# NVlabs/ODISE

Hardware: NVIDIA H100
Metric: images/sec @1024x1024 panoptic inference (ODISE hot path) (higher is better)
Workload: dtype f16q8

## Files before the change

include/odise_b200.h:

```cpp
#ifndef ODISE_B200_H_
#define ODISE_B200_H_

#include <stdint.h>

#ifdef __cplusplus
extern "C" {
#endif

#define ODISE_OK 0
#define ODISE_ERR_ARG 10001
#define ODISE_ERR_ALIGN 10002
#define ODISE_ERR_DRIVER 10003
#define ODISE_ERR_TENSORMAP 10004
#define ODISE_ERR_WORKSPACE 10005
#define ODISE_ERR_UNSUPPORTED 10006

#define ODISE_ACT_NONE 0
#define ODISE_ACT_RELU 1
#define ODISE_ACT_SILU 2
#define ODISE_ACT_GELU 3
#define ODISE_ACT_QUICKGELU 4

#define ODISE_PLANES_BF16 0
#define ODISE_PLANES_F16 1
// ... 77 lines not shown
  float alpha;
  const float* bias;
  const float* rowbias; int rows_per_group; long long rowbias_ld;
  int act;
  const float* residual; long long ld_residual; long long residual_batch_stride;
  float* out_f32; long long ld_out; long long out_batch_stride;
  void* out_hi; void* out_lo; long long ld_out_bf16; long long out_bf16_batch_stride;
  int split_k; void* workspace; long long workspace_bytes;
  int force_bn;
  const float* bias_m;
  int conv_mode;
  int geglu;
  float* gn_partial;
  long long gn_seg_stride; long long gn_plane_stride;
  int out_planes_fp16;
} odise_gemm_desc;
int odise_gemm_bf16(const odise_gemm_desc* desc, void* stream);
int odise_gemm_tile_policy(int M, int N, int K, int batch, int conv3x3, int nmma, int* bn, int* pair);
int odise_profile_begin(void);
int odise_profile_end(long long* launches, double* total_ms, double* total_flops);


int odise_split_f32(const float* x, long long ldx, void* hi, void* lo, long long ldo, long long rows, int cols,
                    void* stream);
int odise_split_f16_f32(const float* x, long long ldx, void* hi, void* lo, long long ldo, long long rows, int cols,
                        void* stream);
int odise_groupnorm_stats_f32(const float* x, long long ldx, float* mean, float* rstd, int B, int HW, int C, int G,
                              float eps, void* stream);
int odise_groupnorm_stats_bs_f32(const float* x, long long ldx, long long x_bs, float* mean, float* rstd, int B,
                                 int HW, int C, int G, float eps, void* stream);
long long odise_groupnorm_ws_floats(int B, int HW, int C, int G);
int odise_groupnorm_stats_ws_f32(const float* x, long long ldx, long long x_bs, float* ws, float* mean, float* rstd,
                                 int B, int HW, int C, int G, float eps, void* stream);
// ... 118 lines not shown
```

odise_b200/csrc/gemm_tc.cu:

```cuda
#include "ptx.cuh"
#include "wgmma.cuh"
#include "odise_b200.h"
#include "launch_count.h"
#include <cudaTypedefs.h>
#include <mutex>
#include <map>
#include <cstring>
#include <vector>
#include <cstdlib>
#include <cstdio>

namespace ob {

struct GemmParams {
  int M, N, K, batch;
  int a_batched, b_batched;
  int conv, C, H, W, bw, bh, bb;
  int nseg;
  int cstride, cpad;
  int tiles_m, tiles_n, splits, kblocks;
  float alpha;
  const float* bias;
  const float* bias_m;
  const float* rowbias;
// ... 162 lines not shown
template <int BN, int NMMA>
struct GemmCfg {
  static constexpr int BM = 128, BK = 64;
  static constexpr int A_BYTES = BM * BK * 2;
  static constexpr int B_BYTES = BN * BK * 2;
  static constexpr int PLANES = (NMMA == 1) ? 1 : 2;
  static constexpr int STAGE_BYTES = PLANES * (A_BYTES + B_BYTES);
  static constexpr int THREADS = 384;
  static constexpr int EPI_BYTES = 8 * 32 * 16 * 4;
  static constexpr int STAGES_RAW = (232448 - EPI_BYTES - 256 - 1024) / STAGE_BYTES;
  static constexpr int STAGES = STAGES_RAW > 8 ? 8 : STAGES_RAW;
  static constexpr int SMEM_BYTES = STAGES * STAGE_BYTES + EPI_BYTES + 256 + 1024;
  static_assert(STAGES >= 2, "GEMM tile does not fit shared memory");
};

template <int BN, int NMMA, int EPI>
__global__ void __launch_bounds__(GemmCfg<BN, NMMA>::THREADS, 1)
gemm_tc_kernel(const __grid_constant__ CUtensorMap tmAh, const __grid_constant__ CUtensorMap tmAl,
               const __grid_constant__ CUtensorMap tmBh, const __grid_constant__ CUtensorMap tmBl, const GemmParams p) {
  using Cfg = GemmCfg<BN, NMMA>;
  extern __shared__ uint8_t smem_raw[];
  uint8_t* smem = reinterpret_cast<uint8_t*>((reinterpret_cast<uintptr_t>(smem_raw) + 1023) & ~uintptr_t(1023));
  float* epi_smem = reinterpret_cast<float*>(smem + Cfg::STAGES * Cfg::STAGE_BYTES);
  uint64_t* bars = reinterpret_cast<uint64_t*>(smem + Cfg::STAGES * Cfg::STAGE_BYTES + Cfg::EPI_BYTES);
  uint64_t* full = bars;
  uint64_t* empty = bars + Cfg::STAGES;

  const int warp = threadIdx.x >> 5;
  const int lane = threadIdx.x & 31;

  if (warp == 8 && lane == 0) {
    tma_prefetch_desc(&tmAh);
    tma_prefetch_desc(&tmBh);
    if (NMMA != 1) {
      tma_prefetch_desc(&tmAl);
      tma_prefetch_desc(&tmBl);
    }
    for (int s = 0; s < Cfg::STAGES; ++s) {
      mbar_init(&full[s], 1);
      mbar_init(&empty[s], 8);
    }
    fence_barrier_init();
  }
  __syncthreads();

  const int tiles_per_z = p.tiles_m * p.tiles_n * p.splits;
  const int total_tiles = tiles_per_z * p.batch;
  const int kb_per_split = (p.kblocks + p.splits - 1) / p.splits;

  if (warp >= 8) {
    setmaxnreg_dec<40>();
    if (warp == 8 && lane == 0) {
      int stage = 0;
      uint32_t phase = 0;
      const int cpk = p.conv ? (p.C / 64) : 1;
      for (int tile = blockIdx.x; tile < total_tiles; tile += gridDim.x) {
        const int z = tile / tiles_per_z;
        int r = tile - z * tiles_per_z;
        const int sp = r / (p.tiles_m * p.tiles_n);
        r -= sp * (p.tiles_m * p.tiles_n);
        const int mt = r / p.tiles_n, nt = r % p.tiles_n;
        const int m0 = mt * 128, n0 = nt * BN;
        const int kb0 = sp * kb_per_split;
        const int kb1 = min(p.kblocks, kb0 + kb_per_split);
        int b0 = 0, h0 = 0, w0 = 0;
        if (p.conv) {
          const int hw = p.H * p.W;
          b0 = m0 / hw;
          const int rem = m0 - b0 * hw;
          h0 = rem / p.W;
          w0 = rem - h0 * p.W;
        }
        for (int kb = kb0; kb < kb1; ++kb) {
          mbar_wait(&empty[stage], phase ^ 1);
          uint8_t* st = smem + stage * Cfg::STAGE_BYTES;
          mbar_arrive_expect_tx(&full[stage], Cfg::STAGE_BYTES);
// ... 4 lines not shown
              const int cx = w0 * p.cstride + kw - p.cpad, cy = h0 * p.cstride + kh - p.cpad;
              tma_load_4d(st, &tmAh, &full[stage], cc * 64, cx, cy, b0);
              if (NMMA != 1) tma_load_4d(st + Cfg::A_BYTES, &tmAl, &full[stage], cc * 64, cx, cy, b0);
            } else {
              const int hw = p.H * p.W;
              for (int sg = 0; sg < p.nseg; ++sg) {
                const int m = m0 + sg * p.bw;
                const int bi = m / hw, rem = m - bi * hw;
                const int hi_ = rem / p.W, wi = rem - hi_ * p.W;
                const int cx = wi * p.cstride + kw - p.cpad, cy = hi_ * p.cstride + kh - p.cpad;
                uint8_t* sa = st + sg * p.bw * 128;
                tma_load_4d(sa, &tmAh, &full[stage], cc * 64, cx, cy, bi);
                if (NMMA != 1) tma_load_4d(sa + Cfg::A_BYTES, &tmAl, &full[stage], cc * 64, cx, cy, bi);
              }
            }
          } else {
            const int za = p.a_batched ? z : 0;
            tma_load_3d(st, &tmAh, &full[stage], kb * 64, m0, za);
            if (NMMA != 1) tma_load_3d(st + Cfg::A_BYTES, &tmAl, &full[stage], kb * 64, m0, za);
          }
          const int zb = p.b_batched ? z : 0;
          uint8_t* sb = st + Cfg::PLANES * Cfg::A_BYTES;
          tma_load_3d(sb, &tmBh, &full[stage], kb * 64, n0, zb);
          if (NMMA != 1) tma_load_3d(sb + Cfg::B_BYTES, &tmBl, &full[stage], kb * 64, n0, zb);
          if (++stage == Cfg::STAGES) { stage = 0; phase ^= 1; }
        }
      }
    }
    return;
  }

  setmaxnreg_inc<232>();
  const int wg = warp >> 2, wi = warp & 3;
  int stage = 0;
  uint32_t phase = 0;
  float acc[BN / 2];
  float acc2[BN / 2];
  float* stg_wg = epi_smem + wg * (4 * 512);
  float* stg = stg_wg + wi * 512;
  const int cq = lane & 3, rsub = lane >> 2;
  for (int tile = blockIdx.x; tile < total_tiles; tile += gridDim.x) {
    const int z = tile / tiles_per_z;
    int r = tile - z * tiles_per_z;
    const int sp = r / (p.tiles_m * p.tiles_n);
    r -= sp * (p.tiles_m * p.tiles_n);
    const int mt = r / p.tiles_n, nt = r % p.tiles_n;
    const int n0 = nt * BN;
    const int kb0 = sp * kb_per_split;
    const int kb1 = min(p.kblocks, kb0 + kb_per_split);

    if (kb0 >= kb1) {
#pragma unroll
      for (int i = 0; i < BN / 2; ++i) acc[i] = 0.f;
      if constexpr (NMMA == 2) {
#pragma unroll
        for (int i = 0; i < BN / 2; ++i) acc2[i] = 0.f;
      }
    }
    int prev = -1;
    for (int kb = kb0; kb < kb1; ++kb) {
      mbar_wait(&full[stage], phase);
// ... 12 lines not shown
        if constexpr (NMMA == 3) {
          wgmma_bf16(acc, a_hi, wgmma_desc_sw128(sb + Cfg::B_BYTES + k * 32), 1);
          wgmma_bf16(acc, wgmma_desc_sw128(sa + Cfg::A_BYTES + k * 32), b_hi, 1);
        }
      }
      if constexpr (NMMA == 2) {
        const uint32_t a2 = sa + Cfg::A_BYTES, b2 = sb + Cfg::B_BYTES;
#pragma unroll
        for (int k = 0; k < 2; ++k) {
          wgmma_e5m2(acc2, wgmma_desc_sw128(a2 + k * 32), wgmma_desc_sw128(b2 + 64 + k * 32), (kb > kb0 || k > 0) ? 1 : 0);
          wgmma_e5m2(acc2, wgmma_desc_sw128(a2 + 64 + k * 32), wgmma_desc_sw128(b2 + k * 32), 1);
        }
      }
      wgmma_commit();
      wgmma_wait<1>();
      if (prev >= 0 && lane == 0) mbar_arrive(&empty[prev]);
      prev = stage;
      if (++stage == Cfg::STAGES) { stage = 0; phase ^= 1; }
    }
    wgmma_wait<0>();
    reg_fence(acc);
    if (prev >= 0 && lane == 0) mbar_arrive(&empty[prev]);
    if constexpr (NMMA == 2) {
      reg_fence(acc2);
#pragma unroll
      for (int i = 0; i < BN / 2; ++i) acc[i] += acc2[i];
    }

    const int m_base = mt * 128 + wg * 64 + (wi & 1) * 32;
    const bool interior = p.vec_ok && p.splits == 1 && (mt * 128 + 128 <= p.M) && (n0 + BN <= p.N);
    constexpr bool EXTRA = EPI == 1, GEGLU = EPI == 2;
    const bool has_bias = p.bias != nullptr, has_res = EXTRA && p.res != nullptr;
    const bool to_f32 = p.D != nullptr, to_hi = p.Dh != nullptr, to_lo = p.Dl != nullptr;
    const int act = p.act;
    const float alpha = p.alpha;
    const bool has_gn = !GEGLU && p.gnp != nullptr;
    const long long gn_seg = ((long long)z * p.M + m_base) >> 5;
// ... 162 lines not shown
  });
  return fn;
}

static int encode_map(CUtensorMap* tm, const void* base, int rank, const cuuint64_t* dims,
                      const cuuint64_t* strides_bytes, const cuuint32_t* box, int spatial_stride = 1) {
  auto enc = get_encode();
  if (!enc) return ODISE_ERR_DRIVER;
  cuuint32_t estr[5] = {1, (cuuint32_t)spatial_stride, (cuuint32_t)spatial_stride, 1, 1};
  CUresult r = enc(tm, CU_TENSOR_MAP_DATA_TYPE_BFLOAT16, rank, const_cast<void*>(base), dims, strides_bytes, box,
                   estr, CU_TENSOR_MAP_INTERLEAVE_NONE, CU_TENSOR_MAP_SWIZZLE_128B,
                   CU_TENSOR_MAP_L2_PROMOTION_L2_256B, CU_TENSOR_MAP_FLOAT_OOB_FILL_NONE);
  return r == CUDA_SUCCESS ? ODISE_OK : ODISE_ERR_TENSORMAP;
}

struct ProfRec { cudaEvent_t a, b; double flops; int M, N, K, batch, conv, bn, nmma, splits; };
static std::vector<ProfRec> g_prof;
static bool g_prof_on = false;

int num_sms() {
  static int n = 0;
  if (!n) {
    int dev = 0;
    cudaGetDevice(&dev);
    cudaDeviceGetAttribute(&n, cudaDevAttrMultiProcessorCount, dev);
    if (n <= 0) n = 132;
  }
  return n;
}

template <int BN, int NMMA, int EPI>
static int launch_cfg(const CUtensorMap& ah, const CUtensorMap& al, const CUtensorMap& bh, const CUtensorMap& bl,
                      const GemmParams& p, cudaStream_t stream) {
  using Cfg = GemmCfg<BN, NMMA>;
  static bool attr_set = false;
  if (!attr_set) {
    cudaError_t e = cudaFuncSetAttribute(gemm_tc_kernel<BN, NMMA, EPI>, cudaFuncAttributeMaxDynamicSharedMemorySize,
                                         Cfg::SMEM_BYTES);
    if (e != cudaSuccess) return (int)e;
    attr_set = true;
  }
  const int total = p.tiles_m * p.tiles_n * p.splits * p.batch;
  const int grid = total < num_sms() ? total : num_sms();
  gemm_tc_kernel<BN, NMMA, EPI><<<grid, Cfg::THREADS, Cfg::SMEM_BYTES, stream>>>(ah, al, bh, bl, p);
  return (int)cudaGetLastError();
}

static int pick_tile(int M, int N, int K, int batch, int forced, bool conv, int nmma) {
  const int cands[4] = {256, 160, 128, 64};
  const double eff[4] = {0.833, 0.933, 1.0, 1.333};
  const double epi_k = 480.0;
  const long long tm = (M + 127) / 128;
  double best = 1e30;
  int c = 128;
  for (int i = 0; i < 4; ++i) {
    const int bn = cands[i];
    if (forced && bn != forced) continue;
    if (nmma == 2 && bn > 128) continue;
    const long long tn = (N + bn - 1) / bn;
    const long long units = tm * tn * batch;
    const long long waves = (units + num_sms() - 1) / num_sms();
    double cost;
    if (conv) {
      cost = (double)waves * bn * eff[i] + 0.02 * bn;
    } else {
      const double mma = (double)bn * K * eff[i], epi = (double)bn * epi_k;
      cost = (double)waves * ((mma > epi ? mma : epi) + 20000.0);
    }
    if (cost < best) { best = cost; c = bn; }
  }
  return c;
}

}

using namespace ob;

extern "C" int odise_gemm_bf16(const odise_gemm_desc* d, void* stream_v) {
  cudaStream_t stream = reinterpret_cast<cudaStream_t>(stream_v);
  if (!d || !d->a_hi || !d->b_hi) return ODISE_ERR_ARG;
  if (d->nmma != 1 && d->nmma != 2 && d->nmma != 3) return ODISE_ERR_ARG;
  if (d->nmma != 1 && (!d->a_lo || !d->b_lo)) return ODISE_ERR_ARG;
  if (d->M <= 0 || d->N <= 0 || d->K <= 0 || d->batch <= 0) return ODISE_ERR_ARG;
  if (!d->out_f32 && !d->out_hi) return ODISE_ERR_ARG;

  GemmParams p{};
  p.M = d->M; p.N = d->N; p.K = d->K; p.batch = d->batch;
  p.a_batched = d->a_batch_stride != 0; p.b_batched = d->b_batch_stride != 0;
  p.conv = d->conv3x3; p.C = d->conv_C; p.H = d->conv_H; p.W = d->conv_W;
  p.alpha = d->alpha;
  p.bias = d->bias; p.bias_m = d->bias_m; p.rowbias = d->rowbias; p.rows_per_group = d->rows_per_group > 0 ? d->rows_per_group : 1;
  p.rowbias_ld = d->rowbias_ld;
  p.res = d->residual; p.ldres = d->ld_residual; p.res_bs = d->residual_batch_stride;
  p.D = d->out_f32; p.ldd = d->ld_out; p.d_bs = d->out_batch_stride;
  p.Dh = reinterpret_cast<__nv_bfloat16*>(d->out_hi); p.Dl = reinterpret_cast<__nv_bfloat16*>(d->out_lo);
  p.ldh = d->ld_out_bf16; p.h_bs = d->out_bf16_batch_stride;
  p.act = d->act;
  p.geglu = d->geglu;
  p.h16 = d->out_planes_fp16 == ODISE_PLANES_F16 ? 1 : 0;
// ... 12 lines not shown
  }

  {
    auto al16 = [](const void* q) { return (reinterpret_cast<uintptr_t>(q) & 15) == 0; };
    bool ok = true;
    if (d->out_f32) ok = ok && d->ld_out % 4 == 0 && d->out_batch_stride % 4 == 0 && al16(d->out_f32);
    if (d->residual) ok = ok && d->ld_residual % 4 == 0 && d->residual_batch_stride % 4 == 0 && al16(d->residual);
    if (d->out_hi) ok = ok && d->ld_out_bf16 % 8 == 0 && d->out_bf16_batch_stride % 8 == 0 && al16(d->out_hi) &&
                        (!d->out_lo || al16(d->out_lo));
    if (d->rowbias) ok = ok && d->rowbias_ld % 4 == 0 && al16(d->rowbias);
    if (d->bias) ok = ok && al16(d->bias);
    p.vec_ok = ok ? 1 : 0;
  }

  CUtensorMap ah, al, bh, bl;
  int rc;
  if (p.conv) {
    if (p.C % 64 || d->K != 9 * p.C || d->batch != 1) return ODISE_ERR_ARG;
    if (d->conv_mode < 0 || d->conv_mode > 2) return ODISE_ERR_ARG;
    p.cstride = d->conv_mode == 0 ? 1 : 2;
    p.cpad = d->conv_mode == 2 ? 0 : 1;
    const int Hin = d->conv_H, Win = d->conv_W;
    if (Hin % p.cstride || Win % p.cstride) return ODISE_ERR_ARG;
    p.H = Hin / p.cstride; p.W = Win / p.cstride;
    const int hw = p.H * p.W;
    if (d->M % hw) return ODISE_ERR_ARG;
    const int B = d->M / hw;
    p.nseg = 1;
    bool boxed = false;
    if (p.W % 128 == 0) {
// ... 15 lines not shown
    }
    const long long pix = d->lda;
    if (pix < p.C || pix % 8) return ODISE_ERR_ALIGN;
    cuuint64_t dims[4] = {(cuuint64_t)p.C, (cuuint64_t)Win, (cuuint64_t)Hin, (cuuint64_t)B};
    cuuint64_t str[3] = {(cuuint64_t)pix * 2, (cuuint64_t)pix * Win * 2, (cuuint64_t)pix * Hin * Win * 2};
    cuuint32_t box[4] = {64, (cuuint32_t)(p.bw * p.cstride), (cuuint32_t)(p.bh * p.cstride), (cuuint32_t)p.bb};
    rc = encode_map(&ah, d->a_hi, 4, dims, str, box, p.cstride);
    if (rc) return rc;
    rc = encode_map(&al, d->nmma != 1 ? d->a_lo : d->a_hi, 4, dims, str, box, p.cstride);
    if (rc) return rc;
  } else {
    if (d->lda % 8 || d->a_batch_stride % 8) return ODISE_ERR_ALIGN;
    const long long bs = d->a_batch_stride ? d->a_batch_stride : (long long)d->M * d->lda;
    cuuint64_t dims[3] = {(cuuint64_t)d->K, (cuuint64_t)d->M, (cuuint64_t)(d->a_batch_stride ? d->batch : 1)};
    cuuint64_t str[2] = {(cuuint64_t)d->lda * 2, (cuuint64_t)bs * 2};
    cuuint32_t box[3] = {64, 128, 1};
    rc = encode_map(&ah, d->a_hi, 3, dims, str, box);
    if (rc) return rc;
    if (d->nmma == 2) {
      dims[0] = (cuuint64_t)((d->K + 63) / 64 * 64);
      if ((long long)dims[0] > d->lda) return ODISE_ERR_ALIGN;
    }
    rc = encode_map(&al, d->nmma != 1 ? d->a_lo : d->a_hi, 3, dims, str, box);
    if (rc) return rc;
  }
  p.tiles_m = (d->M + 127) / 128;
  if (d->ldb % 8 || d->b_batch_stride % 8) return ODISE_ERR_ALIGN;
  if (d->nmma == 2 && (long long)((d->K + 63) / 64 * 64) > d->ldb) return ODISE_ERR_ALIGN;
  if (d->geglu) {
    if (!d->out_hi || d->out_f32 || d->residual || d->rowbias || d->bias_m || d->split_k > 1 || d->N % 16 ||
        !p.vec_ok || d->act != ODISE_ACT_NONE)
      return ODISE_ERR_UNSUPPORTED;
  }
  p.kblocks = (d->K + 63) / 64;
  p.splits = d->split_k > 1 ? d->split_k : 1;
  if (p.splits > p.kblocks) p.splits = p.kblocks;
  if (p.splits > 1) {
    if (!d->workspace ||
        d->workspace_bytes < (long long)p.splits * d->batch * d->M * d->N * (long long)sizeof(float))
      return ODISE_ERR_WORKSPACE;
    p.partial = reinterpret_cast<float*>(d->workspace);
  }
  const int epi = d->geglu ? 2 : ((d->residual || d->rowbias || d->bias_m) ? 1 : 0);

  auto launch_with = [&](int bn) -> int {
    p.tiles_n = (d->N + bn - 1) / bn;
    const long long bs = d->b_batch_stride ? d->b_batch_stride : (long long)d->N * d->ldb;
    cuuint64_t dims[3] = {(cuuint64_t)d->K, (cuuint64_t)d->N, (cuuint64_t)(d->b_batch_stride ? d->batch : 1)};
    cuuint64_t str[2] = {(cuuint64_t)d->ldb * 2, (cuuint64_t)bs * 2};
    cuuint32_t box[3] = {64, (cuuint32_t)bn, 1};
    int r = encode_map(&bh, d->b_hi, 3, dims, str, box);
    if (r) return r;
    if (d->nmma == 2) dims[0] = (cuuint64_t)((d->K + 63) / 64 * 64);
    r = encode_map(&bl, d->nmma != 1 ? d->b_lo : d->b_hi, 3, dims, str, box);
    if (r) return r;
#define ODISE_LAUNCH(BN_, NM_)                                                   \
  r = epi == 2   ? launch_cfg<BN_, NM_, 2>(ah, al, bh, bl, p, stream)            \
      : epi == 1 ? launch_cfg<BN_, NM_, 1>(ah, al, bh, bl, p, stream)            \
                 : launch_cfg<BN_, NM_, 0>(ah, al, bh, bl, p, stream)
    if (d->nmma == 3) {
      switch (bn) {
        case 64: ODISE_LAUNCH(64, 3); break;
        case 128: ODISE_LAUNCH(128, 3); break;
        case 160: ODISE_LAUNCH(160, 3); break;
        default: ODISE_LAUNCH(256, 3); break;
      }
    } else if (d->nmma == 2) {
      if (bn == 64) ODISE_LAUNCH(64, 2);
      else ODISE_LAUNCH(128, 2);
    } else {
      switch (bn) {
        case 64: ODISE_LAUNCH(64, 1); break;
        case 128: ODISE_LAUNCH(128, 1); break;
        case 160: ODISE_LAUNCH(160, 1); break;
        default: ODISE_LAUNCH(256, 1); break;
      }
    }
#undef ODISE_LAUNCH
    if (r) return r;
    if (p.splits > 1) {
      const long long total = (long long)p.batch * p.M * ((p.N + 3) / 4);
      int blocks = (int)((total + 127) / 128);
      if (blocks > num_sms() * 8) blocks = num_sms() * 8;
      gemm_splitk_reduce_kernel<<<blocks, 128, 0, stream>>>(p);
      r = (int)cudaGetLastError();
    }
    return r;
  };

  int BN;
  {
    static const bool tune = !(getenv("ODISE_GEMM_AUTOTUNE") && atoi(getenv("ODISE_GEMM_AUTOTUNE")) == 0);
    const int fbn = (d->force_bn == 64 || d->force_bn == 128 || d->force_bn == 160 || d->force_bn == 256) ? d->force_bn : 0;
    BN = pick_tile(d->M, d->N, d->K, d->batch, fbn, d->conv3x3 != 0, d->nmma);
    struct Key {
      int v[13];
      bool operator<(const Key& o) const { return memcmp(v, o.v, sizeof(v)) < 0; }
    };
    static std::map<Key, int> cache;
    static std::mutex mu;
    const Key key{{d->M, d->N, d->K, d->batch, d->conv3x3 ? 1 + d->conv_mode : 0, d->conv_W, d->nmma, epi, p.splits,
                  (d->out_f32 ? 1 : 0) | (d->out_hi ? 2 : 0) | (d->out_planes_fp16 << 2), p.gnp ? 1 : 0, d->act, p.vec_ok}};
    cudaStreamCaptureStatus cap = cudaStreamCaptureStatusNone;
    cudaStreamIsCapturing(stream, &cap);
    std::lock_guard<std::mutex> lk(mu);
    auto it = cache.find(key);
    if (it != cache.end()) {
      BN = it->second;
    } else if (tune && !fbn && !g_prof_on && cap == cudaStreamCaptureStatusNone &&
               !(d->residual && (const void*)d->residual == (const void*)d->out_f32)) {
      const int cands[4] = {256, 160, 128, 64};
      cudaEvent_t e0, e1;
      cudaEventCreate(&e0);
      cudaEventCreate(&e1);
      float best = 1e30f;
      int bc = BN;
      for (int i = 0; i < 4; ++i) {
        const int c = cands[i];
        if (c == 64 && d->N > 96 && (long long)p.tiles_m * ((d->N + 127) / 128) * d->batch >= 2 * num_sms()) continue;
        if (c > 128 && (d->N <= 64 || d->nmma == 2)) continue;
        if (launch_with(c)) { (void)cudaGetLastError(); continue; }
        cudaEventRecord(e0, stream);
        int r2 = launch_with(c);
        if (!r2) r2 = launch_with(c);
        cudaEventRecord(e1, stream);
        if (r2 || cudaEventSynchronize(e1) != cudaSuccess) { (void)cudaGetLastError(); continue; }
        float ms = 0.f;
        cudaEventElapsedTime(&ms, e0, e1);
        if (ms < best) { best = ms; bc = c; }
      }
      cudaEventDestroy(e0);
      cudaEventDestroy(e1);
      cache[key] = bc;
      BN = bc;
      if (getenv("ODISE_VERBOSE"))
        fprintf(stderr, "odise_b200: gemm %d x %d x %d (batch %d, conv %d, nmma %d, epi %d): BN %d, %.1f us\n", d->M, d->N,
                d->K, d->batch, d->conv3x3, d->nmma, epi, BN, best * 500.f);
    }
  }

  ProfRec rec{};
  if (g_prof_on) {
    cudaEventCreate(&rec.a);
    cudaEventCreate(&rec.b);
    rec.flops = 2.0 * d->M * d->N * (double)d->K * d->batch;
    rec.M = d->M; rec.N = d->N; rec.K = d->K; rec.batch = d->batch; rec.conv = d->conv3x3; rec.bn = BN;
    rec.nmma = d->nmma; rec.splits = p.splits;
    cudaEventRecord(rec.a, stream);
  }
  rc = launch_with(BN);
  if (rc) return rc;
  count_launch(p.splits > 1 ? 2 : 1);
  if (g_prof_on) {
    cudaEventRecord(rec.b, stream);
    g_prof.push_back(rec);
  }
  return rc;
}

extern "C" int odise_gemm_tile_policy(int M, int N, int K, int batch, int conv3x3, int nmma, int* bn, int* pair) {
  if (M <= 0 || N <= 0 || K <= 0 || batch <= 0 || !bn || !pair || nmma < 1 || nmma > 3) return ODISE_ERR_ARG;
  *bn = pick_tile(M, N, K, batch, 0, conv3x3 != 0, nmma);
  *pair = 0;
  return ODISE_OK;
}

extern "C" int odise_profile_begin(void) {
  for (auto& r : g_prof) { cudaEventDestroy(r.a); cudaEventDestroy(r.b); }
  g_prof.clear();
  g_prof_on = true;
  return ODISE_OK;
}

extern "C" int odise_profile_end(long long* launches, double* total_ms, double* total_flops) {
  g_prof_on = false;
  cudaError_t e = cudaDeviceSynchronize();
  if (e != cudaSuccess) return (int)e;
  double ms = 0, fl = 0;
  FILE* fcsv = nullptr;
  if (const char* path = getenv("ODISE_PROFILE_CSV")) fcsv = fopen(path, "a");
  if (fcsv) fprintf(fcsv, "M,N,K,batch,conv,bn,nmma,splits,ms,tflops\n");
  for (auto& r : g_prof) {
    float t = 0;
    cudaEventElapsedTime(&t, r.a, r.b);
    ms += t;
    fl += r.flops;
    if (fcsv)
      fprintf(fcsv, "%d,%d,%d,%d,%d,%d,%d,%d,%.4f,%.1f\n", r.M, r.N, r.K, r.batch, r.conv, r.bn, r.nmma, r.splits, t,
              r.flops / (t * 1e9));
  }
  if (fcsv) fclose(fcsv);
  if (launches) *launches = (long long)g_prof.size();
  if (total_ms) *total_ms = ms;
  if (total_flops) *total_flops = fl;
  for (auto& r : g_prof) { cudaEventDestroy(r.a); cudaEventDestroy(r.b); }
  g_prof.clear();
  return ODISE_OK;
}
```

odise_b200/csrc/ptx.cuh:

```cuda
#pragma once
#include <cuda.h>
#include <cuda_runtime.h>
#include <cuda_bf16.h>
#include <cuda_fp16.h>
#include <cuda_fp8.h>
#include <stdint.h>
#include <stdio.h>

namespace ob {

__device__ __forceinline__ uint32_t smem_u32(const void* p) {
  return static_cast<uint32_t>(__cvta_generic_to_shared(p));
}
__device__ __forceinline__ uint32_t lane_id() { return threadIdx.x & 31; }

__device__ __forceinline__ bool elect_one() {
  uint32_t pred = 0;
  asm volatile(
      "{\n\t.reg .pred P;\n\telect.sync _|P, 0xffffffff;\n\tselp.u32 %0, 1, 0, P;\n\t}\n"
      : "=r"(pred));
  return pred != 0;
}

__device__ __forceinline__ void mbar_init(uint64_t* bar, uint32_t count) {
// ... 40 lines not shown
  asm volatile("prefetch.tensormap [%0];" ::"l"(reinterpret_cast<uint64_t>(m)) : "memory");
}
__device__ __forceinline__ void tma_load_3d(void* smem_dst, const CUtensorMap* m, uint64_t* bar, int c0, int c1,
                                            int c2) {
  asm volatile(
      "cp.async.bulk.tensor.3d.shared::cluster.global.mbarrier::complete_tx::bytes [%0], [%1, {%3, %4, %5}], [%2];"
      ::"r"(smem_u32(smem_dst)), "l"(reinterpret_cast<uint64_t>(m)), "r"(smem_u32(bar)), "r"(c0), "r"(c1), "r"(c2)
      : "memory");
}
__device__ __forceinline__ void tma_load_4d(void* smem_dst, const CUtensorMap* m, uint64_t* bar, int c0, int c1,
                                            int c2, int c3) {
  asm volatile(
      "cp.async.bulk.tensor.4d.shared::cluster.global.mbarrier::complete_tx::bytes [%0], [%1, {%3, %4, %5, %6}], "
      "[%2];" ::"r"(smem_u32(smem_dst)),
      "l"(reinterpret_cast<uint64_t>(m)), "r"(smem_u32(bar)), "r"(c0), "r"(c1), "r"(c2), "r"(c3)
      : "memory");
}

__device__ __forceinline__ void named_bar_sync(uint32_t id, uint32_t threads) {
  asm volatile("bar.sync %0, %1;" ::"r"(id), "r"(threads) : "memory");
}
__device__ __forceinline__ void wgmma_fence() { asm volatile("wgmma.fence.sync.aligned;" ::: "memory"); }
__device__ __forceinline__ void wgmma_commit() { asm volatile("wgmma.commit_group.sync.aligned;" ::: "memory"); }
template <int N>
__device__ __forceinline__ void wgmma_wait() {
  asm volatile("wgmma.wait_group.sync.aligned %0;" ::"n"(N) : "memory");
}
template <int R>
__device__ __forceinline__ void reg_fence(float (&d)[R]) {
#pragma unroll
// ... 113 lines not shown
```

odise_b200/lib.py:

```python
import ctypes
import os
from ctypes import c_int, c_float, c_longlong, c_void_p, POINTER

import torch

_HERE = os.path.dirname(os.path.abspath(__file__))
_LIB_PATH = os.path.join(_HERE, "libodise_b200.so")

ACT_NONE, ACT_RELU, ACT_SILU, ACT_GELU, ACT_QUICKGELU = 0, 1, 2, 3, 4


class OdiseError(RuntimeError):
    pass


class GemmDesc(ctypes.Structure):
    _fields_ = [
        ("M", c_int), ("N", c_int), ("K", c_int), ("batch", c_int),
        ("nmma", c_int), ("conv3x3", c_int),
        ("conv_C", c_int), ("conv_H", c_int), ("conv_W", c_int),
        ("a_hi", c_void_p), ("a_lo", c_void_p), ("lda", c_longlong), ("a_batch_stride", c_longlong),
        ("b_hi", c_void_p), ("b_lo", c_void_p), ("ldb", c_longlong), ("b_batch_stride", c_longlong),
        ("alpha", c_float),
        ("bias", c_void_p),
        ("rowbias", c_void_p), ("rows_per_group", c_int), ("rowbias_ld", c_longlong),
        ("act", c_int),
        ("residual", c_void_p), ("ld_residual", c_longlong), ("residual_batch_stride", c_longlong),
        ("out_f32", c_void_p), ("ld_out", c_longlong), ("out_batch_stride", c_longlong),
        ("out_hi", c_void_p), ("out_lo", c_void_p), ("ld_out_bf16", c_longlong), ("out_bf16_batch_stride", c_longlong),
        ("split_k", c_int), ("workspace", c_void_p), ("workspace_bytes", c_longlong),
        ("force_bn", c_int),
        ("bias_m", c_void_p),
        ("conv_mode", c_int),
        ("geglu", c_int),
        ("gn_partial", c_void_p), ("gn_seg_stride", c_longlong), ("gn_plane_stride", c_longlong),
        ("out_planes_fp16", c_int),
    ]


_lib = None

_SIGS = {
    "odise_msda_forward_f32": [c_void_p] * 6 + [c_int] * 7 + [c_void_p],
    "odise_msda_fused_f32": [c_void_p] * 9 + [c_int] * 7 + [c_void_p],
    "odise_msda_forward_f64": [c_void_p] * 6 + [c_int] * 7 + [c_void_p],
    "odise_msda_backward_f32": [c_void_p] * 9 + [c_int] * 7 + [c_void_p],
    "odise_msda_backward_f64": [c_void_p] * 9 + [c_int] * 7 + [c_void_p],
    "odise_msda_fused_backward_f32": [c_void_p] * 10 + [c_int] * 7 + [c_void_p],
    "odise_msda_fused_f16": [c_void_p] * 7 + [c_int] * 7 + [c_void_p],
    "odise_msda_fused_bf16": [c_void_p] * 7 + [c_int] * 7 + [c_void_p],
    "odise_msda_fused_backward_f16": [c_void_p] * 10 + [c_int] * 7 + [c_void_p],
    "odise_msda_fused_backward_bf16": [c_void_p] * 10 + [c_int] * 7 + [c_void_p],
    "odise_msda_det_workspace_bytes": [c_int] * 4,
    "odise_msda_backward_det_f32": [c_void_p] * 9 + [c_int] * 7 + [c_void_p, c_void_p],
    "odise_msda_backward_det_f64": [c_void_p] * 9 + [c_int] * 7 + [c_void_p, c_void_p],
    "odise_msda_fused_backward_det_f32": [c_void_p] * 10 + [c_int] * 7 + [c_void_p, c_void_p],
    "odise_msda_fused_backward_det_f16": [c_void_p] * 10 + [c_int] * 7 + [c_void_p, c_void_p],
    "odise_msda_fused_backward_det_bf16": [c_void_p] * 10 + [c_int] * 7 + [c_void_p, c_void_p],
    "odise_gemm_bf16": [POINTER(GemmDesc), c_void_p],
    "odise_gemm_tile_policy": [c_int] * 6 + [c_void_p, c_void_p],
    "odise_profile_begin": [],
    "odise_profile_end": [c_void_p, c_void_p, c_void_p],
    "odise_split_f32": [c_void_p, c_longlong, c_void_p, c_void_p, c_longlong, c_longlong, c_int, c_void_p],
    "odise_split_f16_f32": [c_void_p, c_longlong, c_void_p, c_void_p, c_longlong, c_longlong, c_int, c_void_p],
    "odise_groupnorm_stats_f32": [c_void_p, c_longlong, c_void_p, c_void_p, c_int, c_int, c_int, c_int, c_float,
                                  c_void_p],
    "odise_groupnorm_apply_f32": [c_void_p, c_longlong, c_void_p, c_void_p, c_void_p, c_void_p, c_int, c_void_p,
                                  c_longlong, c_void_p, c_void_p, c_longlong, c_int, c_int, c_int, c_int, c_void_p],
    "odise_groupnorm_finalize_seg_f32": [c_void_p, c_longlong, c_longlong, c_void_p, c_void_p, c_int, c_int, c_int, c_int,
                                         c_float, c_void_p],
    "odise_groupnorm_stats_bs_f32": [c_void_p, c_longlong, c_longlong, c_void_p, c_void_p, c_int, c_int, c_int, c_int,
                                     c_float, c_void_p],
    "odise_groupnorm_stats_ws_f32": [c_void_p, c_longlong, c_longlong, c_void_p, c_void_p, c_void_p, c_int, c_int,
                                     c_int, c_int, c_float, c_void_p],
    "odise_groupnorm_apply_bs_f32": [c_void_p, c_longlong, c_longlong, c_void_p, c_void_p, c_void_p, c_void_p, c_int,
# ... 270 lines not shown


def conv_ok(H, W):
    import math
    if W % 128 == 0:
        return True
    if 128 % W == 0:
        bh = min(128 // W, H)
        if H % bh == 0 and 128 % (W * bh) == 0:
            return True
    return math.gcd(W, 128) % 8 == 0


def gemm(a, b, *, M=None, N=None, K=None, nmma=3, batch=1, a_bs=0, b_bs=0, conv=None, alpha=1.0, bias=None, bias_m=None,
         rowbias=None, rows_per_group=1, act=ACT_NONE, residual=None, ld_res=None, res_bs=0, out=None, ld_out=None,
         out_bs=0, out_planes=None, outp_bs=0, split_k=1, workspace=None, force_bn=0, geglu=False, conv_mode=0, gn=None):
    d = GemmDesc()
    d.M = M if M is not None else a.rows
    d.N = N if N is not None else b.rows
    d.K = K if K is not None else (9 * conv[0] if conv else a.cols)
    d.batch = batch
    if conv:
        d.conv3x3, d.conv_C, d.conv_H, d.conv_W = 1, conv[0], conv[1], conv[2]
    if a.f16 or b.f16:
        raise OdiseError("gemm: fp16 planes are attention-kernel operands (V^T), not GEMM inputs")
    if a.fmt != b.fmt:
        raise OdiseError(f"gemm: operand formats differ ({a.fmt} x {b.fmt})")
    if a.fmt == "q8":
        if nmma == 1:
            raise OdiseError("gemm: F16Q8 operands have no plain-bf16 mode")
        nmma = 2
# ... 15 lines not shown
    if out is not None:
        d.out_f32 = _ptr(out)
        d.ld_out = ld_out if ld_out is not None else out.stride(-2)
        d.out_batch_stride = out_bs
    if out_planes is not None:
        d.out_hi, d.out_lo, d.ld_out_bf16 = _ptr(out_planes.hi), _ptr(out_planes.lo), out_planes.ld
        d.out_bf16_batch_stride = outp_bs
        d.out_planes_fp16 = out_planes.code
    d.split_k = split_k
    if split_k > 1:
        need = split_k * batch * d.M * d.N * 4
        if workspace is None or workspace.numel() * workspace.element_size() < need:
            raise OdiseError("gemm: split_k needs a workspace of %d bytes" % need)
        d.workspace, d.workspace_bytes = _ptr(workspace), workspace.numel() * workspace.element_size()
    d.force_bn = force_bn
    if gn is not None:
        if split_k > 1 or gn.missing or d.M % 32 or gn.C != d.N or gn.rows != d.M * batch:
            gn.missing = True
        else:
            d.gn_partial = gn.ptr
            d.gn_seg_stride, d.gn_plane_stride = 3 * gn.Ctot, gn.Ctot
    d.geglu = 1 if geglu else 0
    d.conv_mode = conv_mode
    _check(load().odise_gemm_bf16(ctypes.byref(d), _stream()), "odise_gemm_bf16")
    return out if out is not None else out_planes


def gemm_tile_policy(M, N, K, batch=1, conv=False, nmma=2):
    bn, pair = c_int(0), c_int(0)
    _check(load().odise_gemm_tile_policy(M, N, K, batch, 1 if conv else 0, nmma, ctypes.byref(bn), ctypes.byref(pair)),
           "odise_gemm_tile_policy")
    return bn.value, bool(pair.value)


def msda_forward(value, spatial_shapes, level_start_index, sampling_locations, attention_weights, im2col_step=128):
    for t, nm in ((value, "value"), (sampling_locations, "sampling_loc"), (attention_weights, "attn_weight")):
        if not t.is_cuda:
            raise OdiseError(f"{nm} must be a CUDA tensor")
        if not t.is_contiguous():
            raise OdiseError(f"{nm} tensor has to be contiguous")
        _req(t, torch.float32, nm)
    N, S, M, D = value.shape
    _, Lq, _, L, P, _ = sampling_locations.shape
    step = min(N, im2col_step)
    if N % step != 0:
        raise OdiseError(f"batch({N}) must divide im2col_step({step})")
    ss = spatial_shapes.to(device=value.device, dtype=torch.int64).contiguous()
# ... 203 lines not shown
```

Measured before the change: 9.966.

## Add 2-CTA thread-block clusters with TMA multicast to the GEMM kernel

```diff
diff --git a/include/odise_b200.h b/include/odise_b200.h
--- a/include/odise_b200.h
+++ b/include/odise_b200.h
@@ -115,9 +115,11 @@
   float* gn_partial;
   long long gn_seg_stride; long long gn_plane_stride;
   int out_planes_fp16;
+  int force_cluster;
 } odise_gemm_desc;
 int odise_gemm_bf16(const odise_gemm_desc* desc, void* stream);
 int odise_gemm_tile_policy(int M, int N, int K, int batch, int conv3x3, int nmma, int* bn, int* pair);
+int odise_gemm_cluster_policy(int M, int N, int K, int batch, int conv3x3, int nmma, int* cm, int* cn);
 int odise_profile_begin(void);
 int odise_profile_end(long long* launches, double* total_ms, double* total_flops);
 
diff --git a/odise_b200/csrc/gemm_tc.cu b/odise_b200/csrc/gemm_tc.cu
--- a/odise_b200/csrc/gemm_tc.cu
+++ b/odise_b200/csrc/gemm_tc.cu
@@ -200,11 +200,12 @@
   static_assert(STAGES >= 2, "GEMM tile does not fit shared memory");
 };
 
-template <int BN, int NMMA, int EPI>
+template <int BN, int NMMA, int EPI, int CM, int CN>
 __global__ void __launch_bounds__(GemmCfg<BN, NMMA>::THREADS, 1)
 gemm_tc_kernel(const __grid_constant__ CUtensorMap tmAh, const __grid_constant__ CUtensorMap tmAl,
                const __grid_constant__ CUtensorMap tmBh, const __grid_constant__ CUtensorMap tmBl, const GemmParams p) {
   using Cfg = GemmCfg<BN, NMMA>;
+  constexpr int CS = CM * CN;
   extern __shared__ uint8_t smem_raw[];
   uint8_t* smem = reinterpret_cast<uint8_t*>((reinterpret_cast<uintptr_t>(smem_raw) + 1023) & ~uintptr_t(1023));
   float* epi_smem = reinterpret_cast<float*>(smem + Cfg::STAGES * Cfg::STAGE_BYTES);
@@ -224,13 +225,17 @@
     }
     for (int s = 0; s < Cfg::STAGES; ++s) {
       mbar_init(&full[s], 1);
-      mbar_init(&empty[s], 8);
+      mbar_init(&empty[s], 8 * CS);
     }
     fence_barrier_init();
   }
-  __syncthreads();
-
-  const int tiles_per_z = p.tiles_m * p.tiles_n * p.splits;
+  if constexpr (CS > 1) cluster_sync();
+  else __syncthreads();
+
+  const int crank = CS > 1 ? (int)cluster_ctarank() : 0;
+  const int rm = crank % CM, rn = crank / CM;
+  const int ctiles_m = (p.tiles_m + CM - 1) / CM, ctiles_n = (p.tiles_n + CN - 1) / CN;
+  const int tiles_per_z = ctiles_m * ctiles_n * p.splits;
   const int total_tiles = tiles_per_z * p.batch;
   const int kb_per_split = (p.kblocks + p.splits - 1) / p.splits;
 
@@ -240,12 +245,12 @@
       int stage = 0;
       uint32_t phase = 0;
       const int cpk = p.conv ? (p.C / 64) : 1;
-      for (int tile = blockIdx.x; tile < total_tiles; tile += gridDim.x) {
+      for (int tile = blockIdx.x / CS; tile < total_tiles; tile += gridDim.x / CS) {
         const int z = tile / tiles_per_z;
         int r = tile - z * tiles_per_z;
-        const int sp = r / (p.tiles_m * p.tiles_n);
-        r -= sp * (p.tiles_m * p.tiles_n);
-        const int mt = r / p.tiles_n, nt = r % p.tiles_n;
+        const int sp = r / (ctiles_m * ctiles_n);
+        r -= sp * (ctiles_m * ctiles_n);
+        const int mt = (r / ctiles_n) * CM + rm, nt = (r % ctiles_n) * CN + rn;
         const int m0 = mt * 128, n0 = nt * BN;
         const int kb0 = sp * kb_per_split;
         const int kb1 = min(p.kblocks, kb0 + kb_per_split);
@@ -280,15 +285,38 @@
                 if (NMMA != 1) tma_load_4d(sa + Cfg::A_BYTES, &tmAl, &full[stage], cc * 64, cx, cy, bi);
               }
             }
-          } else {
+          } else if constexpr (CN == 1) {
             const int za = p.a_batched ? z : 0;
             tma_load_3d(st, &tmAh, &full[stage], kb * 64, m0, za);
             if (NMMA != 1) tma_load_3d(st + Cfg::A_BYTES, &tmAl, &full[stage], kb * 64, m0, za);
+          } else {
+            constexpr int AR = 128 / CN;
+            uint16_t mask = 0;
+#pragma unroll
+            for (int j = 0; j < CN; ++j) mask |= (uint16_t)(1u << (rm + j * CM));
+            const int za = p.a_batched ? z : 0;
+            tma_load_3d_mc(st + rn * AR * 128, &tmAh, &full[stage], kb * 64, m0 + rn * AR, za, mask);
+            if (NMMA != 1)
+              tma_load_3d_mc(st + Cfg::A_BYTES + rn * AR * 128, &tmAl, &full[stage], kb * 64, m0 + rn * AR, za, mask);
           }
           const int zb = p.b_batched ? z : 0;
           uint8_t* sb = st + Cfg::PLANES * Cfg::A_BYTES;
-          tma_load_3d(sb, &tmBh, &full[stage], kb * 64, n0, zb);
-          if (NMMA != 1) tma_load_3d(sb + Cfg::B_BYTES, &tmBl, &full[stage], kb * 64, n0, zb);
+          if constexpr (CM == 1) {
+            tma_load_3d(sb, &tmBh, &full[stage], kb * 64, n0, zb);
+            if (NMMA != 1) tma_load_3d(sb + Cfg::B_BYTES, &tmBl, &full[stage], kb * 64, n0, zb);
+          } else {
+            constexpr int BR = BN / CM;
+            const uint16_t mask = (uint16_t)(((1u << CM) - 1) << (rn * CM));
+            tma_load_3d_mc(sb + rm * BR * 128, &tmBh, &full[stage], kb * 64, n0 + rm * BR, zb, mask);
+            if (NMMA != 1)
+              tma_load_3d_mc(sb + Cfg::B_BYTES + rm * BR * 128, &tmBl, &full[stage], kb * 64, n0 + rm * BR, zb, mask);
+          }
+          if (++stage == Cfg::STAGES) { stage = 0; phase ^= 1; }
+        }
+      }
+      if constexpr (CS > 1) {
+        for (int s = 0; s < Cfg::STAGES; ++s) {
+          mbar_wait(&empty[stage], phase ^ 1);
           if (++stage == Cfg::STAGES) { stage = 0; phase ^= 1; }
         }
       }
@@ -305,12 +333,20 @@
   float* stg_wg = epi_smem + wg * (4 * 512);
   float* stg = stg_wg + wi * 512;
   const int cq = lane & 3, rsub = lane >> 2;
-  for (int tile = blockIdx.x; tile < total_tiles; tile += gridDim.x) {
+  auto release = [&](int s) {
+    if constexpr (CS == 1) {
+      mbar_arrive(&empty[s]);
+    } else {
+#pragma unroll
+      for (int c = 0; c < CS; ++c) mbar_arrive_cluster(&empty[s], c);
+    }
+  };
+  for (int tile = blockIdx.x / CS; tile < total_tiles; tile += gridDim.x / CS) {
     const int z = tile / tiles_per_z;
     int r = tile - z * tiles_per_z;
-    const int sp = r / (p.tiles_m * p.tiles_n);
-    r -= sp * (p.tiles_m * p.tiles_n);
-    const int mt = r / p.tiles_n, nt = r % p.tiles_n;
+    const int sp = r / (ctiles_m * ctiles_n);
+    r -= sp * (ctiles_m * ctiles_n);
+    const int mt = (r / ctiles_n) * CM + rm, nt = (r % ctiles_n) * CN + rn;
     const int n0 = nt * BN;
     const int kb0 = sp * kb_per_split;
     const int kb1 = min(p.kblocks, kb0 + kb_per_split);
@@ -353,13 +389,16 @@
       }
       wgmma_commit();
       wgmma_wait<1>();
-      if (prev >= 0 && lane == 0) mbar_arrive(&empty[prev]);
+      if (prev >= 0 && lane == 0) release(prev);
       prev = stage;
       if (++stage == Cfg::STAGES) { stage = 0; phase ^= 1; }
     }
     wgmma_wait<0>();
     reg_fence(acc);
-    if (prev >= 0 && lane == 0) mbar_arrive(&empty[prev]);
+    if (prev >= 0 && lane == 0) release(prev);
+    if constexpr (CS > 1) {
+      if (mt >= p.tiles_m || nt >= p.tiles_n) continue;
+    }
     if constexpr (NMMA == 2) {
       reg_fence(acc2);
 #pragma unroll
@@ -552,7 +591,7 @@
   return r == CUDA_SUCCESS ? ODISE_OK : ODISE_ERR_TENSORMAP;
 }
 
-struct ProfRec { cudaEvent_t a, b; double flops; int M, N, K, batch, conv, bn, nmma, splits; };
+struct ProfRec { cudaEvent_t a, b; double flops; int M, N, K, batch, conv, bn, nmma, splits, cl; };
 static std::vector<ProfRec> g_prof;
 static bool g_prof_on = false;
 
@@ -567,20 +606,46 @@
   return n;
 }
 
-template <int BN, int NMMA, int EPI>
+template <int BN, int NMMA, int EPI, int CM, int CN>
 static int launch_cfg(const CUtensorMap& ah, const CUtensorMap& al, const CUtensorMap& bh, const CUtensorMap& bl,
                       const GemmParams& p, cudaStream_t stream) {
   using Cfg = GemmCfg<BN, NMMA>;
+  constexpr int CS = CM * CN;
+  auto kern = gemm_tc_kernel<BN, NMMA, EPI, CM, CN>;
   static bool attr_set = false;
   if (!attr_set) {
-    cudaError_t e = cudaFuncSetAttribute(gemm_tc_kernel<BN, NMMA, EPI>, cudaFuncAttributeMaxDynamicSharedMemorySize,
-                                         Cfg::SMEM_BYTES);
+    cudaError_t e = cudaFuncSetAttribute(kern, cudaFuncAttributeMaxDynamicSharedMemorySize, Cfg::SMEM_BYTES);
     if (e != cudaSuccess) return (int)e;
     attr_set = true;
   }
-  const int total = p.tiles_m * p.tiles_n * p.splits * p.batch;
-  const int grid = total < num_sms() ? total : num_sms();
-  gemm_tc_kernel<BN, NMMA, EPI><<<grid, Cfg::THREADS, Cfg::SMEM_BYTES, stream>>>(ah, al, bh, bl, p);
+  if constexpr (CS == 1) {
+    const int total = p.tiles_m * p.tiles_n * p.splits * p.batch;
+    const int grid = total < num_sms() ? total : num_sms();
+    kern<<<grid, Cfg::THREADS, Cfg::SMEM_BYTES, stream>>>(ah, al, bh, bl, p);
+  } else {
+    cudaLaunchAttribute attr[1];
+    attr[0].id = cudaLaunchAttributeClusterDimension;
+    attr[0].val.clusterDim.x = CS;
+    attr[0].val.clusterDim.y = 1;
+    attr[0].val.clusterDim.z = 1;
+    cudaLaunchConfig_t cfg = {};
+    cfg.blockDim = dim3(Cfg::THREADS);
+    cfg.dynamicSmemBytes = Cfg::SMEM_BYTES;
+    cfg.stream = stream;
+    cfg.attrs = attr;
+    cfg.numAttrs = 1;
+    static int max_clusters = 0;
+    if (!max_clusters) {
+      cfg.gridDim = dim3(num_sms() / CS * CS);
+      cudaError_t e = cudaOccupancyMaxActiveClusters(&max_clusters, kern, &cfg);
+      if (e != cudaSuccess) return (int)e;
+      if (max_clusters <= 0) return ODISE_ERR_UNSUPPORTED;
+    }
+    const int ctiles = (p.tiles_m + CM - 1) / CM * ((p.tiles_n + CN - 1) / CN) * p.splits * p.batch;
+    cfg.gridDim = dim3((ctiles < max_clusters ? ctiles : max_clusters) * CS);
+    cudaError_t e = cudaLaunchKernelEx(&cfg, kern, ah, al, bh, bl, p);
+    if (e != cudaSuccess) return (int)e;
+  }
   return (int)cudaGetLastError();
 }
 
@@ -610,6 +675,17 @@
   return c;
 }
 
+static int pick_cluster(int M, int N, int batch, bool conv, int bn) {
+  const long long tm = (M + 127) / 128, tn = (N + bn - 1) / bn, sms = num_sms(), pairs = sms / 2;
+  double best = (double)((tm * tn * batch + sms - 1) / sms);
+  int c = 1;
+  const double mpair = 0.75 * (double)(((tm + 1) / 2 * tn * batch + pairs - 1) / pairs);
+  if (tm >= 2 && mpair < best) { best = mpair; c = 2; }
+  const double npair = 0.75 * (double)((tm * ((tn + 1) / 2) * batch + pairs - 1) / pairs);
+  if (!conv && tn >= 2 && npair < best) c = 3;
+  return c;
+}
+
 }
 
 using namespace ob;
@@ -621,6 +697,8 @@
   if (d->nmma != 1 && (!d->a_lo || !d->b_lo)) return ODISE_ERR_ARG;
   if (d->M <= 0 || d->N <= 0 || d->K <= 0 || d->batch <= 0) return ODISE_ERR_ARG;
   if (!d->out_f32 && !d->out_hi) return ODISE_ERR_ARG;
+  if (d->force_cluster < 0 || d->force_cluster > 3) return ODISE_ERR_ARG;
+  if (d->force_cluster == 3 && d->conv3x3) return ODISE_ERR_UNSUPPORTED;
 
   GemmParams p{};
   p.M = d->M; p.N = d->N; p.K = d->K; p.batch = d->batch;
@@ -663,6 +741,7 @@
   }
 
   CUtensorMap ah, al, bh, bl;
+  CUtensorMap ah_half, al_half;
   int rc;
   if (p.conv) {
     if (p.C % 64 || d->K != 9 * p.C || d->batch != 1) return ODISE_ERR_ARG;
@@ -708,14 +787,16 @@
     const long long bs = d->a_batch_stride ? d->a_batch_stride : (long long)d->M * d->lda;
     cuuint64_t dims[3] = {(cuuint64_t)d->K, (cuuint64_t)d->M, (cuuint64_t)(d->a_batch_stride ? d->batch : 1)};
     cuuint64_t str[2] = {(cuuint64_t)d->lda * 2, (cuuint64_t)bs * 2};
-    cuuint32_t box[3] = {64, 128, 1};
+    cuuint32_t box[3] = {64, 128, 1}, half[3] = {64, 64, 1};
     rc = encode_map(&ah, d->a_hi, 3, dims, str, box);
+    if (!rc) rc = encode_map(&ah_half, d->a_hi, 3, dims, str, half);
     if (rc) return rc;
     if (d->nmma == 2) {
       dims[0] = (cuuint64_t)((d->K + 63) / 64 * 64);
       if ((long long)dims[0] > d->lda) return ODISE_ERR_ALIGN;
     }
     rc = encode_map(&al, d->nmma != 1 ? d->a_lo : d->a_hi, 3, dims, str, box);
+    if (!rc) rc = encode_map(&al_half, d->nmma != 1 ? d->a_lo : d->a_hi, 3, dims, str, half);
     if (rc) return rc;
   }
   p.tiles_m = (d->M + 127) / 128;
@@ -737,21 +818,25 @@
   }
   const int epi = d->geglu ? 2 : ((d->residual || d->rowbias || d->bias_m) ? 1 : 0);
 
-  auto launch_with = [&](int bn) -> int {
+  auto launch_with = [&](int bn, int cl) -> int {
     p.tiles_n = (d->N + bn - 1) / bn;
     const long long bs = d->b_batch_stride ? d->b_batch_stride : (long long)d->N * d->ldb;
     cuuint64_t dims[3] = {(cuuint64_t)d->K, (cuuint64_t)d->N, (cuuint64_t)(d->b_batch_stride ? d->batch : 1)};
     cuuint64_t str[2] = {(cuuint64_t)d->ldb * 2, (cuuint64_t)bs * 2};
-    cuuint32_t box[3] = {64, (cuuint32_t)bn, 1};
+    cuuint32_t box[3] = {64, (cuuint32_t)(cl == 2 ? bn / 2 : bn), 1};
     int r = encode_map(&bh, d->b_hi, 3, dims, str, box);
     if (r) return r;
     if (d->nmma == 2) dims[0] = (cuuint64_t)((d->K + 63) / 64 * 64);
     r = encode_map(&bl, d->nmma != 1 ? d->b_lo : d->b_hi, 3, dims, str, box);
     if (r) return r;
-#define ODISE_LAUNCH(BN_, NM_)                                                   \
-  r = epi == 2   ? launch_cfg<BN_, NM_, 2>(ah, al, bh, bl, p, stream)            \
-      : epi == 1 ? launch_cfg<BN_, NM_, 1>(ah, al, bh, bl, p, stream)            \
-                 : launch_cfg<BN_, NM_, 0>(ah, al, bh, bl, p, stream)
+#define ODISE_LAUNCH_EPI(BN_, NM_, CM_, CN_, AH, AL)                                         \
+  (epi == 2   ? launch_cfg<BN_, NM_, 2, CM_, CN_>(AH, AL, bh, bl, p, stream)                 \
+   : epi == 1 ? launch_cfg<BN_, NM_, 1, CM_, CN_>(AH, AL, bh, bl, p, stream)                 \
+              : launch_cfg<BN_, NM_, 0, CM_, CN_>(AH, AL, bh, bl, p, stream))
+#define ODISE_LAUNCH(BN_, NM_)                                                               \
+  r = cl == 2   ? ODISE_LAUNCH_EPI(BN_, NM_, 2, 1, ah, al)                                   \
+      : cl == 3 ? ODISE_LAUNCH_EPI(BN_, NM_, 1, 2, ah_half, al_half)                         \
+                : ODISE_LAUNCH_EPI(BN_, NM_, 1, 1, ah, al)
     if (d->nmma == 3) {
       switch (bn) {
         case 64: ODISE_LAUNCH(64, 3); break;
@@ -771,6 +856,7 @@
       }
     }
 #undef ODISE_LAUNCH
+#undef ODISE_LAUNCH_EPI
     if (r) return r;
     if (p.splits > 1) {
       const long long total = (long long)p.batch * p.M * ((p.N + 3) / 4);
@@ -782,16 +868,18 @@
     return r;
   };
 
-  int BN;
+  int BN, CL;
   {
     static const bool tune = !(getenv("ODISE_GEMM_AUTOTUNE") && atoi(getenv("ODISE_GEMM_AUTOTUNE")) == 0);
     const int fbn = (d->force_bn == 64 || d->force_bn == 128 || d->force_bn == 160 || d->force_bn == 256) ? d->force_bn : 0;
+    const int fcl = d->force_cluster;
     BN = pick_tile(d->M, d->N, d->K, d->batch, fbn, d->conv3x3 != 0, d->nmma);
+    CL = pick_cluster(d->M, d->N, d->batch, d->conv3x3 != 0, BN);
     struct Key {
       int v[13];
       bool operator<(const Key& o) const { return memcmp(v, o.v, sizeof(v)) < 0; }
     };
-    static std::map<Key, int> cache;
+    static std::map<Key, std::pair<int, int>> cache;
     static std::mutex mu;
     const Key key{{d->M, d->N, d->K, d->batch, d->conv3x3 ? 1 + d->conv_mode : 0, d->conv_W, d->nmma, epi, p.splits,
                   (d->out_f32 ? 1 : 0) | (d->out_hi ? 2 : 0) | (d->out_planes_fp16 << 2), p.gnp ? 1 : 0, d->act, p.vec_ok}};
@@ -800,37 +888,44 @@
     std::lock_guard<std::mutex> lk(mu);
     auto it = cache.find(key);
     if (it != cache.end()) {
-      BN = it->second;
-    } else if (tune && !fbn && !g_prof_on && cap == cudaStreamCaptureStatusNone &&
+      BN = it->second.first;
+      CL = it->second.second;
+    } else if (tune && !fbn && !fcl && !g_prof_on && cap == cudaStreamCaptureStatusNone &&
                !(d->residual && (const void*)d->residual == (const void*)d->out_f32)) {
       const int cands[4] = {256, 160, 128, 64};
       cudaEvent_t e0, e1;
       cudaEventCreate(&e0);
       cudaEventCreate(&e1);
       float best = 1e30f;
-      int bc = BN;
+      int bc = BN, bcl = CL;
       for (int i = 0; i < 4; ++i) {
         const int c = cands[i];
         if (c == 64 && d->N > 96 && (long long)p.tiles_m * ((d->N + 127) / 128) * d->batch >= 2 * num_sms()) continue;
         if (c > 128 && (d->N <= 64 || d->nmma == 2)) continue;
-        if (launch_with(c)) { (void)cudaGetLastError(); continue; }
-        cudaEventRecord(e0, stream);
-        int r2 = launch_with(c);
-        if (!r2) r2 = launch_with(c);
-        cudaEventRecord(e1, stream);
-        if (r2 || cudaEventSynchronize(e1) != cudaSuccess) { (void)cudaGetLastError(); continue; }
-        float ms = 0.f;
-        cudaEventElapsedTime(&ms, e0, e1);
-        if (ms < best) { best = ms; bc = c; }
+        for (int cl = 1; cl <= 3; ++cl) {
+          if (cl == 2 && p.tiles_m < 2) continue;
+          if (cl == 3 && (d->conv3x3 || d->N <= c)) continue;
+          if (launch_with(c, cl)) { (void)cudaGetLastError(); continue; }
+          cudaEventRecord(e0, stream);
+          int r2 = launch_with(c, cl);
+          if (!r2) r2 = launch_with(c, cl);
+          cudaEventRecord(e1, stream);
+          if (r2 || cudaEventSynchronize(e1) != cudaSuccess) { (void)cudaGetLastError(); continue; }
+          float ms = 0.f;
+          cudaEventElapsedTime(&ms, e0, e1);
+          if (ms < best) { best = ms; bc = c; bcl = cl; }
+        }
       }
       cudaEventDestroy(e0);
       cudaEventDestroy(e1);
-      cache[key] = bc;
+      cache[key] = {bc, bcl};
       BN = bc;
+      CL = bcl;
       if (getenv("ODISE_VERBOSE"))
-        fprintf(stderr, "odise_b200: gemm %d x %d x %d (batch %d, conv %d, nmma %d, epi %d): BN %d, %.1f us\n", d->M, d->N,
-                d->K, d->batch, d->conv3x3, d->nmma, epi, BN, best * 500.f);
-    }
+        fprintf(stderr, "odise_b200: gemm %d x %d x %d (batch %d, conv %d, nmma %d, epi %d): BN %d, cluster %d, %.1f us\n",
+                d->M, d->N, d->K, d->batch, d->conv3x3, d->nmma, epi, BN, CL, best * 500.f);
+    }
+    if (fcl) CL = fcl;
   }
 
   ProfRec rec{};
@@ -839,10 +934,10 @@
     cudaEventCreate(&rec.b);
     rec.flops = 2.0 * d->M * d->N * (double)d->K * d->batch;
     rec.M = d->M; rec.N = d->N; rec.K = d->K; rec.batch = d->batch; rec.conv = d->conv3x3; rec.bn = BN;
-    rec.nmma = d->nmma; rec.splits = p.splits;
+    rec.nmma = d->nmma; rec.splits = p.splits; rec.cl = CL;
     cudaEventRecord(rec.a, stream);
   }
-  rc = launch_with(BN);
+  rc = launch_with(BN, CL);
   if (rc) return rc;
   count_launch(p.splits > 1 ? 2 : 1);
   if (g_prof_on) {
@@ -856,6 +951,14 @@
   if (M <= 0 || N <= 0 || K <= 0 || batch <= 0 || !bn || !pair || nmma < 1 || nmma > 3) return ODISE_ERR_ARG;
   *bn = pick_tile(M, N, K, batch, 0, conv3x3 != 0, nmma);
   *pair = 0;
+  return ODISE_OK;
+}
+
+extern "C" int odise_gemm_cluster_policy(int M, int N, int K, int batch, int conv3x3, int nmma, int* cm, int* cn) {
+  if (M <= 0 || N <= 0 || K <= 0 || batch <= 0 || !cm || !cn || nmma < 1 || nmma > 3) return ODISE_ERR_ARG;
+  const int cl = pick_cluster(M, N, batch, conv3x3 != 0, pick_tile(M, N, K, batch, 0, conv3x3 != 0, nmma));
+  *cm = cl == 2 ? 2 : 1;
+  *cn = cl == 3 ? 2 : 1;
   return ODISE_OK;
 }
 
@@ -873,15 +976,15 @@
   double ms = 0, fl = 0;
   FILE* fcsv = nullptr;
   if (const char* path = getenv("ODISE_PROFILE_CSV")) fcsv = fopen(path, "a");
-  if (fcsv) fprintf(fcsv, "M,N,K,batch,conv,bn,nmma,splits,ms,tflops\n");
+  if (fcsv) fprintf(fcsv, "M,N,K,batch,conv,bn,nmma,splits,ms,tflops,cluster\n");
   for (auto& r : g_prof) {
     float t = 0;
     cudaEventElapsedTime(&t, r.a, r.b);
     ms += t;
     fl += r.flops;
     if (fcsv)
-      fprintf(fcsv, "%d,%d,%d,%d,%d,%d,%d,%d,%.4f,%.1f\n", r.M, r.N, r.K, r.batch, r.conv, r.bn, r.nmma, r.splits, t,
-              r.flops / (t * 1e9));
+      fprintf(fcsv, "%d,%d,%d,%d,%d,%d,%d,%d,%.4f,%.1f,%d\n", r.M, r.N, r.K, r.batch, r.conv, r.bn, r.nmma, r.splits, t,
+              r.flops / (t * 1e9), r.cl);
   }
   if (fcsv) fclose(fcsv);
   if (launches) *launches = (long long)g_prof.size();
diff --git a/odise_b200/csrc/ptx.cuh b/odise_b200/csrc/ptx.cuh
--- a/odise_b200/csrc/ptx.cuh
+++ b/odise_b200/csrc/ptx.cuh
@@ -78,6 +78,31 @@
       "cp.async.bulk.tensor.4d.shared::cluster.global.mbarrier::complete_tx::bytes [%0], [%1, {%3, %4, %5, %6}], "
       "[%2];" ::"r"(smem_u32(smem_dst)),
       "l"(reinterpret_cast<uint64_t>(m)), "r"(smem_u32(bar)), "r"(c0), "r"(c1), "r"(c2), "r"(c3)
+      : "memory");
+}
+
+__device__ __forceinline__ uint32_t cluster_ctarank() {
+  uint32_t r;
+  asm volatile("mov.u32 %0, %%cluster_ctarank;" : "=r"(r));
+  return r;
+}
+__device__ __forceinline__ void cluster_sync() {
+  asm volatile("barrier.cluster.arrive.release.aligned;\n\tbarrier.cluster.wait.acquire.aligned;" ::: "memory");
+}
+__device__ __forceinline__ void mbar_arrive_cluster(uint64_t* bar, uint32_t cta) {
+  asm volatile(
+      "{\n\t.reg .b32 ra;\n\t"
+      "mapa.shared::cluster.u32 ra, %0, %1;\n\t"
+      "mbarrier.arrive.shared::cluster.b64 _, [ra];\n\t}" ::"r"(smem_u32(bar)),
+      "r"(cta)
+      : "memory");
+}
+__device__ __forceinline__ void tma_load_3d_mc(void* smem_dst, const CUtensorMap* m, uint64_t* bar, int c0, int c1,
+                                               int c2, uint16_t mask) {
+  asm volatile(
+      "cp.async.bulk.tensor.3d.shared::cluster.global.mbarrier::complete_tx::bytes.multicast::cluster [%0], [%1, {%3, "
+      "%4, %5}], [%2], %6;" ::"r"(smem_u32(smem_dst)),
+      "l"(reinterpret_cast<uint64_t>(m)), "r"(smem_u32(bar)), "r"(c0), "r"(c1), "r"(c2), "h"(mask)
       : "memory");
 }
 
diff --git a/odise_b200/lib.py b/odise_b200/lib.py
--- a/odise_b200/lib.py
+++ b/odise_b200/lib.py
@@ -35,6 +35,7 @@
         ("geglu", c_int),
         ("gn_partial", c_void_p), ("gn_seg_stride", c_longlong), ("gn_plane_stride", c_longlong),
         ("out_planes_fp16", c_int),
+        ("force_cluster", c_int),
     ]
 
 
@@ -59,6 +60,7 @@
     "odise_msda_fused_backward_det_bf16": [c_void_p] * 10 + [c_int] * 7 + [c_void_p, c_void_p],
     "odise_gemm_bf16": [POINTER(GemmDesc), c_void_p],
     "odise_gemm_tile_policy": [c_int] * 6 + [c_void_p, c_void_p],
+    "odise_gemm_cluster_policy": [c_int] * 6 + [c_void_p, c_void_p],
     "odise_profile_begin": [],
     "odise_profile_end": [c_void_p, c_void_p, c_void_p],
     "odise_split_f32": [c_void_p, c_longlong, c_void_p, c_void_p, c_longlong, c_longlong, c_int, c_void_p],
@@ -359,7 +361,8 @@
 
 def gemm(a, b, *, M=None, N=None, K=None, nmma=3, batch=1, a_bs=0, b_bs=0, conv=None, alpha=1.0, bias=None, bias_m=None,
          rowbias=None, rows_per_group=1, act=ACT_NONE, residual=None, ld_res=None, res_bs=0, out=None, ld_out=None,
-         out_bs=0, out_planes=None, outp_bs=0, split_k=1, workspace=None, force_bn=0, geglu=False, conv_mode=0, gn=None):
+         out_bs=0, out_planes=None, outp_bs=0, split_k=1, workspace=None, force_bn=0, geglu=False, conv_mode=0, gn=None,
+         force_cluster=0):
     d = GemmDesc()
     d.M = M if M is not None else a.rows
     d.N = N if N is not None else b.rows
@@ -405,6 +408,7 @@
             raise OdiseError("gemm: split_k needs a workspace of %d bytes" % need)
         d.workspace, d.workspace_bytes = _ptr(workspace), workspace.numel() * workspace.element_size()
     d.force_bn = force_bn
+    d.force_cluster = force_cluster
     if gn is not None:
         if split_k > 1 or gn.missing or d.M % 32 or gn.C != d.N or gn.rows != d.M * batch:
             gn.missing = True
@@ -422,6 +426,13 @@
     _check(load().odise_gemm_tile_policy(M, N, K, batch, 1 if conv else 0, nmma, ctypes.byref(bn), ctypes.byref(pair)),
            "odise_gemm_tile_policy")
     return bn.value, bool(pair.value)
+
+
+def gemm_cluster_policy(M, N, K, batch=1, conv=False, nmma=2):
+    cm, cn = c_int(0), c_int(0)
+    _check(load().odise_gemm_cluster_policy(M, N, K, batch, 1 if conv else 0, nmma, ctypes.byref(cm), ctypes.byref(cn)),
+           "odise_gemm_cluster_policy")
+    return cm.value, cn.value
 
 
 def msda_forward(value, spatial_shapes, level_start_index, sampling_locations, attention_weights, im2col_step=128):
```

New measurement: 10.11, median of 6. 1.01x the previous value.
